# dusk-network/dusk-blindbidproof

Hardware: AMD Instinct MI355X
Metric: blind-bid proofs/sec (higher is better)
Workload: dtype u32

## Files before the change

__graft_entry__.py:

```python
import os
import shutil
import subprocess
import sys

ROOT = os.path.dirname(os.path.abspath(__file__))
PKG = os.path.join(ROOT, "dusk_blindbidproof_amd")
CSRC = os.path.join(PKG, "csrc")
LIB = os.path.join(PKG, "libbbp_hip.so")
ORACLE_SO = os.path.join(ROOT, "oracle", "_build", "libbbp_oracle.so")
HOSTCHECK_SO = os.path.join(ROOT, "tests", "_build", "libhostcheck.so")
DEVCHECK_SO = {"chain": os.path.join(ROOT, "tests", "_build", "libbbp_devcheck.so"),
               "nochain": os.path.join(ROOT, "tests", "_build", "libbbp_devcheck_nochain.so")}
DEVCHECK_DEFS = {"chain": [], "nochain": ["-DBBP_FE_NO_CHAIN"]}


def _newer(target, sources):
    if not os.path.exists(target):
        return True
    t = os.path.getmtime(target)
    return any(os.path.getmtime(s) > t for s in sources)


def _run(cmd):
    print("+", " ".join(cmd), flush=True)
# ... 169 lines not shown
    src = os.path.join(ROOT, "tests", "wire_fuzz.cpp")
    sdir = os.path.join(PKG, "server")
    if force or _newer(WIRE_FUZZ_BIN, [src, os.path.join(sdir, "wire.h"), os.path.join(sdir, "tlv.h")]):
        os.makedirs(os.path.dirname(WIRE_FUZZ_BIN), exist_ok=True)
        _run(["g++", "-O1", "-g", "-std=c++17", "-fsanitize=address,undefined", "-fno-sanitize-recover=all", "-o", WIRE_FUZZ_BIN, src])
    return WIRE_FUZZ_BIN


VERIFY_PLAN_SAN_BIN = os.path.join(ROOT, "tests", "_build", "verify_plan_san")


def build_verify_plan_san(force=False):
    src = os.path.join(ROOT, "tests", "verify_plan_san.cpp")
    if force or _newer(VERIFY_PLAN_SAN_BIN, [src, os.path.join(ROOT, "tests", "host_check.cpp")] + _csrc_files((".h", ".inc"))):
        os.makedirs(os.path.dirname(VERIFY_PLAN_SAN_BIN), exist_ok=True)
        _run(["g++", "-O1", "-g", "-std=c++17", "-fsanitize=address,undefined", "-fno-sanitize-recover=all", "-o", VERIFY_PLAN_SAN_BIN, src])
    return VERIFY_PLAN_SAN_BIN


BATCH_LAYOUT_SAN_BIN = os.path.join(ROOT, "tests", "_build", "batch_layout_san")


def build_batch_layout_san(force=False):
    src = os.path.join(ROOT, "tests", "batch_layout_san.cpp")
    if force or _newer(BATCH_LAYOUT_SAN_BIN, [src, os.path.join(ROOT, "tests", "host_check.cpp")] + _csrc_files((".h", ".inc"))):
        os.makedirs(os.path.dirname(BATCH_LAYOUT_SAN_BIN), exist_ok=True)
        _run(["g++", "-O1", "-g", "-std=c++17", "-fsanitize=address,undefined", "-fno-sanitize-recover=all", "-o", BATCH_LAYOUT_SAN_BIN, src])
    return BATCH_LAYOUT_SAN_BIN


HEDGE_SAN_BIN = os.path.join(ROOT, "tests", "_build", "hedge_san")


def build_hedge_san(force=False):
    src = os.path.join(ROOT, "tests", "hedge_san.cpp")
    if force or _newer(HEDGE_SAN_BIN, [src] + _csrc_files((".h", ".inc"))):
        os.makedirs(os.path.dirname(HEDGE_SAN_BIN), exist_ok=True)
        _run(["g++", "-O1", "-g", "-std=c++17", "-fsanitize=address,undefined", "-fno-sanitize-recover=all", "-o", HEDGE_SAN_BIN, src])
    return HEDGE_SAN_BIN


TAIL_SHARE_BIN = os.path.join(ROOT, "tests", "_build", "tail_share_check")


def build_tail_share_check(force=False):
    src = os.path.join(ROOT, "tests", "tail_share_check.cpp")
    if force or _newer(TAIL_SHARE_BIN, [src] + _csrc_files((".h", ".inc"))):
        os.makedirs(os.path.dirname(TAIL_SHARE_BIN), exist_ok=True)
        _run(["g++", "-O1", "-g", "-std=c++17", "-fsanitize=address,undefined", "-fno-sanitize=signed-integer-overflow,shift", "-fno-sanitize-recover=all", "-o",
              TAIL_SHARE_BIN, src])
    return TAIL_SHARE_BIN


SECRET_MAP_BIN = os.path.join(ROOT, "tests", "_build", "secret_map_check")
SECRET_WIPE_SAN_BIN = os.path.join(ROOT, "tests", "_build", "secret_wipe_san")


def build_secret_map_check(force=False):
    src = os.path.join(ROOT, "tests", "secret_map_check.cpp")
    if force or _newer(SECRET_MAP_BIN, [src] + _csrc_files((".h", ".inc"))):
        os.makedirs(os.path.dirname(SECRET_MAP_BIN), exist_ok=True)
        _run(["g++", "-O1", "-g", "-std=c++17", "-fsanitize=address,undefined", "-fno-sanitize-recover=all", "-o", SECRET_MAP_BIN, src])
    return SECRET_MAP_BIN


ROUND_SELECT_BIN = os.path.join(ROOT, "tests", "_build", "round_select_check")


def build_round_select_check(force=False):
    src = os.path.join(ROOT, "tests", "round_select_check.cpp")
    if force or _newer(ROUND_SELECT_BIN, [src] + _csrc_files((".h", ".inc")) + [os.path.join(ROOT, "include", "bbp.h")]):
        os.makedirs(os.path.dirname(ROUND_SELECT_BIN), exist_ok=True)
        _run(["g++", "-O1", "-g", "-std=c++17", "-fsanitize=address,undefined", "-fno-sanitize-recover=all", "-o", ROUND_SELECT_BIN, src])
    return ROUND_SELECT_BIN


ROUND_BEST_BIN = os.path.join(ROOT, "tests", "_build", "round_best_check")


def build_round_best_check(force=False):
    src = os.path.join(ROOT, "tests", "round_best_check.cpp")
    if force or _newer(ROUND_BEST_BIN, [src] + _csrc_files((".h", ".inc")) + [os.path.join(ROOT, "include", "bbp.h")]):
        os.makedirs(os.path.dirname(ROUND_BEST_BIN), exist_ok=True)
        _run(["g++", "-O1", "-g", "-std=c++17", "-fsanitize=address,undefined", "-fno-sanitize-recover=all", "-o", ROUND_BEST_BIN, src])
    return ROUND_BEST_BIN


ROUNDS_BEST_BIN = os.path.join(ROOT, "tests", "_build", "rounds_best_check")


def build_rounds_best_check(force=False):
    src = os.path.join(ROOT, "tests", "rounds_best_check.cpp")
    if force or _newer(ROUNDS_BEST_BIN, [src] + _csrc_files((".h", ".inc")) + [os.path.join(ROOT, "include", "bbp.h")]):
        os.makedirs(os.path.dirname(ROUNDS_BEST_BIN), exist_ok=True)
        _run(["g++", "-O1", "-g", "-std=c++17", "-fsanitize=address,undefined", "-fno-sanitize-recover=all", "-o", ROUNDS_BEST_BIN, src])
    return ROUNDS_BEST_BIN


ROUND_BEST_DISTINCT_BIN = os.path.join(ROOT, "tests", "_build", "round_best_distinct_check")


def build_round_best_distinct_check(force=False):
    src = os.path.join(ROOT, "tests", "round_best_distinct_check.cpp")
    if force or _newer(ROUND_BEST_DISTINCT_BIN, [src] + _csrc_files((".h", ".inc")) + [os.path.join(ROOT, "include", "bbp.h")]):
        os.makedirs(os.path.dirname(ROUND_BEST_DISTINCT_BIN), exist_ok=True)
        _run(["g++", "-O1", "-g", "-std=c++17", "-fsanitize=address,undefined", "-fno-sanitize-recover=all", "-o", ROUND_BEST_DISTINCT_BIN, src])
# ... 66 lines not shown
COMBINER_RULES_BIN = os.path.join(ROOT, "tests", "_build", "combiner_rules")


def build_combiner_rules(force=False):
    srcs = [os.path.join(ROOT, "tests", "combiner_rules.cpp"), os.path.join(CSRC, "submit.cpp")]
    if force or _newer(COMBINER_RULES_BIN, srcs + [os.path.join(CSRC, "submit.h")]):
        os.makedirs(os.path.dirname(COMBINER_RULES_BIN), exist_ok=True)
        _run(["g++", "-O1", "-std=c++17", "-pthread", "-o", COMBINER_RULES_BIN] + srcs)
    return COMBINER_RULES_BIN


COMBINER_MIXED_BIN = {False: os.path.join(ROOT, "tests", "_build", "combiner_mixed"), True: os.path.join(ROOT, "tests", "_build", "combiner_mixed_tsan")}


def build_combiner_mixed(tsan=False, force=False):
    out = COMBINER_MIXED_BIN[bool(tsan)]
    srcs = [os.path.join(ROOT, "tests", "combiner_mixed.cpp"), os.path.join(CSRC, "submit.cpp")]
    if force or _newer(out, srcs + [os.path.join(CSRC, "submit.h")]):
        os.makedirs(os.path.dirname(out), exist_ok=True)
        flags = ["-O1", "-g", "-fsanitize=thread"] if tsan else ["-O1"]
        _run(["g++"] + flags + ["-std=c++17", "-pthread", "-o", out] + srcs)
    return out


COMBINER_ROUNDS_BIN = {False: os.path.join(ROOT, "tests", "_build", "combiner_rounds"), True: os.path.join(ROOT, "tests", "_build", "combiner_rounds_tsan")}


def build_combiner_rounds(tsan=False, force=False):
    out = COMBINER_ROUNDS_BIN[bool(tsan)]
    srcs = [os.path.join(ROOT, "tests", "combiner_rounds.cpp"), os.path.join(CSRC, "submit.cpp")]
    if force or _newer(out, srcs + [os.path.join(CSRC, "submit.h")]):
        os.makedirs(os.path.dirname(out), exist_ok=True)
        flags = ["-O1", "-g", "-fsanitize=thread"] if tsan else ["-O1"]
        _run(["g++"] + flags + ["-std=c++17", "-pthread", "-o", out] + srcs)
    return out


def build():
    build_hip()
    build_server()
    build_stub_engine()
    build_oracle()
    build_hostcheck()
    build_sortcheck()
    build_roundcheck()
    build_round_select_check()
    build_round_best_check()
    build_round_best_distinct_check()
    build_rounds_best_check()
    build_rounds_best_distinct_check()
    build_round_standing_check()
    build_standings_check()
    build_tail_share_check()
    build_devcheck_all()
    sys.path.insert(0, ROOT)
    import dusk_blindbidproof_amd


def smoke():
    sys.path.insert(0, ROOT)
    import dusk_blindbidproof_amd as bbp
    from tests import smoke_case

    smoke_case.run(bbp)


if __name__ == "__main__":
    build()
```

dusk_blindbidproof_amd/csrc/keccak.h:

```cpp
#pragma once
#include "field.h"

namespace bbp {

BBP_HD u64 rotl64(u64 x, int n) {
    n &= 63;
    if (n == 0) return x;
#if defined(__HIP_DEVICE_COMPILE__)
    const u32 lo = (u32)x, hi = (u32)(x >> 32);
    if (n == 32) return ((u64)lo << 32) | hi;
    const u32 a = n < 32 ? lo : hi, b = n < 32 ? hi : lo;
    const u32 s = 32u - ((u32)n & 31u);
    const u32 rl = __builtin_amdgcn_alignbit(a, b, s), rh = __builtin_amdgcn_alignbit(b, a, s);
    return ((u64)rh << 32) | rl;
#else
    return (x << n) | (x >> (64 - n));
#endif
}

#define BBP_BITOP3_XOR3 0x96
#define BBP_BITOP3_CHI 0xd2
BBP_HD u64 keccak_xor3(u64 a, u64 b, u64 c) {
#if defined(__HIP_DEVICE_COMPILE__)
    const u32 lo = __builtin_amdgcn_bitop3_b32((u32)a, (u32)b, (u32)c, BBP_BITOP3_XOR3);
// ... 179 lines not shown
BBP_HD void merlin_challenge(merlin_transcript& t, const uint8_t* label, u32 llen, uint8_t* out, u32 n) {
    uint8_t len4[4];
    le32(len4, n);
    strobe_meta_ad(t, label, llen, false);
    strobe_meta_ad(t, len4, 4, true);
    strobe_prf(t, out, n, false);
}

BBP_HD void merlin_rng_rekey(merlin_transcript& t, const uint8_t* label, u32 llen, const uint8_t* w, u32 wlen) {
    uint8_t len4[4];
    le32(len4, wlen);
    strobe_meta_ad(t, label, llen, false);
    strobe_meta_ad(t, len4, 4, true);
    strobe_key(t, w, wlen, false);
}

BBP_HD void merlin_rng_finalize(merlin_transcript& t, const uint8_t* ent32) {
    const uint8_t l[3] = {'r', 'n', 'g'};
    strobe_meta_ad(t, l, 3, false);
    strobe_key(t, ent32, 32, false);
}

BBP_HD void merlin_rng_fill(merlin_transcript& t, uint8_t* out, u32 n) {
    uint8_t len4[4];
    le32(len4, n);
    strobe_meta_ad(t, len4, 4, false);
    strobe_prf(t, out, n, false);
}

BBP_HD bool merlin_rng_fill64_bulk(merlin_transcript& t, u32 count, u32* out_words ) {
    if (t.pos != 64 || t.pos_begin != 0) return false;
    u64 a[25];
#pragma unroll
    for (int i = 0; i < 25; i++) a[i] = t.st[i];
    for (u32 c = 0; c < count; c++) {
        a[8] ^= 0x0741000000401200ull;
        a[9] ^= 0x0000000000000447ull;
        a[20] ^= 0x8000000000000000ull;
        keccak_f1600_body(a);
        u32* o = out_words + (size_t)c * 16;
#pragma unroll
        for (int i = 0; i < 8; i++) {
            o[2 * i] = (u32)a[i];
            o[2 * i + 1] = (u32)(a[i] >> 32);
            a[i] = 0;
        }
    }
#pragma unroll
    for (int i = 0; i < 25; i++) t.st[i] = a[i];
    t.cur_flags = BBP_FLAG_I | BBP_FLAG_A | BBP_FLAG_C;
    return true;
}

}
```

dusk_blindbidproof_amd/csrc/prove_plan.h:

```cpp
#pragma once
#include <stdint.h>
#include <stdio.h>
#include <stdlib.h>
#include <string.h>

#include <string>

namespace bbp {

constexpr int FOLD_ROUND = 7;
constexpr int PROVE_MAX_SLICES = 4;
#ifndef BBP_PROVE_BUFS
#define BBP_PROVE_BUFS 5
#endif
constexpr int PROVE_BUFS = BBP_PROVE_BUFS;

struct ProveKnobs {
    int slices = 3;
    int rotate_below = 1023;
    int rotate_deep_max = 4096;
    int deep_from = 3;
    int mixed_from = 512;
    int dual_open_below = 1024;
    int rng_coop = -1;
    int rng_coop_below = 768;
    int rng_coop_idle_below = 2300;
    int rng_dpp = 2;
    int rng_block = 0;
    int serial_block = 64;
    int serial_lds = 160 * 1024;
    int tr_wave_below = 32;
    int ipa_wide_below = 32;
    int commit_split_below = 1024;
    int witness_native = 1;
    int tail_small_below = 65;
    int tail_round = FOLD_ROUND;
    int stagger_mode = 0;
    int trace_prove = 0;
    int open_on_chain = -1;
    int hw_queues = 4;

    struct Env {
        const char* name;
        int ProveKnobs::*member;
        int (*clamp)(int);
    };
    template <class F>
    static void each_env(F&& f) {
        static const Env table[] = {
            {"BBP_SLICES", &ProveKnobs::slices, [](int v) { return v < 1 ? 1 : v > PROVE_MAX_SLICES ? PROVE_MAX_SLICES : v; }},
            {"BBP_ROTATE_BELOW", &ProveKnobs::rotate_below, nullptr},
            {"BBP_ROTATE_DEEP_MAX", &ProveKnobs::rotate_deep_max, nullptr},
            {"BBP_ROTATE_DEEP_FROM", &ProveKnobs::deep_from, [](int v) { return v < 2 ? 2 : v; }},
            {"BBP_ROTATE_MIXED_FROM", &ProveKnobs::mixed_from, nullptr},
            {"BBP_DUAL_OPEN_BELOW", &ProveKnobs::dual_open_below, nullptr},
            {"BBP_RNG_COOP", &ProveKnobs::rng_coop, [](int v) { return v != 0 ? 1 : 0; }},
            {"BBP_RNG_COOP_BELOW", &ProveKnobs::rng_coop_below, nullptr},
            {"BBP_RNG_COOP_IDLE_BELOW", &ProveKnobs::rng_coop_idle_below, nullptr},
            {"BBP_RNG_DPP", &ProveKnobs::rng_dpp, nullptr},
            {"BBP_RNG_BLOCK", &ProveKnobs::rng_block, [](int v) { return v >= 1024 ? 1024 : v >= 512 ? 512 : v >= 256 ? 256 : v >= 128 ? 128 : 64; }},
            {"BBP_SERIAL_BLOCK", &ProveKnobs::serial_block, [](int v) { return v == 64 ? 64 : v == 128 ? 128 : 256; }},
            {"BBP_SERIAL_LDS", &ProveKnobs::serial_lds, [](int v) { return v < 0 ? 0 : v > 160 * 1024 ? 160 * 1024 : v; }},
            {"BBP_TR_WAVE_BELOW", &ProveKnobs::tr_wave_below, nullptr},
            {"BBP_IPA_WIDE_BELOW", &ProveKnobs::ipa_wide_below, nullptr},
            {"BBP_COMMIT_SPLIT_BELOW", &ProveKnobs::commit_split_below, nullptr},
            {"BBP_WITNESS_NATIVE", &ProveKnobs::witness_native, [](int v) { return v != 0 ? 1 : 0; }},
            {"BBP_TAIL_SMALL_BELOW", &ProveKnobs::tail_small_below, nullptr},
            {"BBP_TAIL_ROUND", &ProveKnobs::tail_round, [](int v) { return v == FOLD_ROUND ? FOLD_ROUND : 12; }},
// ... 35 lines not shown

struct HeavyPlan {
    uint32_t tw = 0;
    uint32_t tgrid = 0;
    bool wide_ipa = false;
    bool split_T = false;
    uint32_t tail_from = 12;
    int stagger_after = 0;
};

inline HeavyPlan plan_heavy(const ProveKnobs& k, uint32_t B) {
    HeavyPlan h;
    h.tw = B <= (uint32_t)k.tr_wave_below ? 1u : 0u;
    h.tgrid = h.tw ? B : (B + 63) / 64;
    h.wide_ipa = B <= (uint32_t)k.ipa_wide_below;
    h.split_T = B * 5 <= (uint32_t)k.commit_split_below;
    h.tail_from = B < (uint32_t)(k.tail_small_below > 0 ? k.tail_small_below : 0) ? 12u : (uint32_t)k.tail_round;
    h.stagger_after = k.stagger_mode;
    return h;
}

enum StreamRole { ROLE_CALLER = 0, ROLE_SIDE, ROLE_LANE1, ROLE_LANE2, ROLE_LANE3, ROLE_COPY, ROLE_SIDE2, ROLE_COUNT };

struct ProvePlan {
    enum Chain { SERIAL, LANES25, WORD, HALFWORD };
    uint32_t call = 0;
    bool deep = false;
    bool behind_sliced = false;
    bool dual = false;
    int open_stream = 0;
    int par = 0;
    bool coop = false;
    Chain chain = SERIAL;
    uint32_t prefix_form = 0;
    uint32_t serial_blk = 64;
    uint32_t cblk = 64;
    bool rotate = false;
    int heavy_stream = 0;
    uint32_t slices = 0;
    bool open_on_chain = false;
    int chain_stream = -1;

    int open_role() const { return open_on_chain ? chain_stream : open_stream ? ROLE_SIDE2 : ROLE_SIDE; }
    int heavy_role() const { return open_on_chain ? chain_stream : ROLE_LANE1 + heavy_stream - 1; }
    static int slice_role(uint32_t i) { return i == 0 ? ROLE_CALLER : ROLE_LANE1 + (int)i - 1; }
    uint32_t roles() const {
        uint32_t mask = 1u << ROLE_CALLER | 1u << open_role();
        if (rotate) mask |= 1u << heavy_role();
        for (uint32_t i = 0; i < slices; i++) mask |= 1u << slice_role(i);
        return mask;
    }
    int raw_index() const { return !open_on_chain ? open_stream : chain_stream == ROLE_SIDE ? 0 : 1 + heavy_stream; }
    uint32_t cblk_wave() const { return 2 * cblk > 1024u ? 1024u : 2 * cblk; }
    uint32_t slice_first(uint32_t B, uint32_t i) const { return (uint32_t)(((uint64_t)B * i) / slices); }

    std::string trace_line(uint32_t call_, uint32_t B, int inflight) const {
        char buf[160];
        snprintf(buf, sizeof buf, "prove call %u: B %u inflight %d deep %d behind_sliced %d dual %d rotate %d par %d coop %d\n", call_, B, inflight,
                 (int)deep, (int)behind_sliced, (int)dual, (int)rotate, par, (int)coop);
        return buf;
    }
};

template <class Busy>
ProvePlan plan_prove(const ProveKnobs& k, ProveRuleState& st, uint32_t B, int inflight, Busy&& sliced_busy) {
    ProvePlan p;
    p.call = st.calls++;
    if (inflight >= k.deep_from) {
        st.deep_mode = true;
        st.deep_idle_seen = 0;
    } else if (++st.deep_idle_seen >= 6) {
        st.deep_mode = false;
    }
    p.deep = (st.deep_mode || st.force_deep) && k.deep_eligible(B);
    p.behind_sliced = !p.deep && k.mixed_from > 0 && B >= (uint32_t)k.mixed_from && st.last_sliced && sliced_busy();
    p.dual = !p.behind_sliced && (p.deep || B < (uint32_t)(k.dual_open_below > 0 ? k.dual_open_below : 0));
    p.open_stream = p.dual ? (int)(p.call & 1u) : 0;
    p.par = p.dual ? (int)(p.call % (uint32_t)PROVE_BUFS) : (int)(p.call & 1u);
    p.coop = k.rng_coop < 0 ? B <= (uint32_t)k.rng_coop_below || (inflight == 0 && B <= (uint32_t)k.rng_coop_idle_below) : k.rng_coop != 0;
    p.chain = !p.coop ? ProvePlan::SERIAL : k.rng_dpp >= 2 ? ProvePlan::HALFWORD : k.rng_dpp ? ProvePlan::WORD : ProvePlan::LANES25;
    p.prefix_form = !p.coop ? 0u : B <= (uint32_t)k.tr_wave_below ? 2u : 1u;
    p.serial_blk = k.serial_lds > 0 ? (uint32_t)k.serial_block : 64u;
    p.cblk = k.rng_block > 0 ? (uint32_t)k.rng_block : (B <= 128 ? 64u : B <= 256 ? 128u : 256u);
    p.rotate = p.dual && ((k.rotate_below > 0 && B <= (uint32_t)k.rotate_below) || (p.deep && B > (uint32_t)k.rotate_below));
    p.heavy_stream = p.rotate ? 1 + (int)(p.call % (uint32_t)(PROVE_MAX_SLICES - 1)) : 0;
    p.slices = B >= 64u * (uint32_t)k.slices ? (uint32_t)k.slices : (B >= 128 ? 2u : 1u);
    if (p.dual && p.slices > 2) p.slices = 2;
    if (p.rotate) p.slices = 0;
    p.open_on_chain = p.rotate && k.chain_rule(p.deep);
    p.chain_stream = !p.open_on_chain ? -1 : p.heavy_stream == 3 ? (int)ROLE_SIDE : (int)ROLE_LANE1 + p.heavy_stream - 1;
    return p;
}

}
```

dusk_blindbidproof_amd/csrc/prover.hip:

```cpp
#define BBP_KECCAK_WAVE 1
#include <string.h>

#include <functional>

#include "batch.h"
#include "hosthash.h"
#include "keccak_wave.h"
#include "scalarmul.h"
#include "witness.h"

namespace bbp {

#define BBP_THIN_PRIO() __builtin_amdgcn_s_setprio(3)
#ifndef BBP_LANE_KERNEL
#define BBP_LANE_KERNEL __launch_bounds__(64)
#endif


__device__ __forceinline__ void sc_to_bytes32(uint8_t* o, const sc& s) { sc_tobytes(o, s); }
__device__ __forceinline__ void words_to_bytes32(uint8_t* o, const u32* w) {
#pragma unroll
    for (int i = 0; i < 8; i++) {
        o[4 * i] = (uint8_t)w[i];
        o[4 * i + 1] = (uint8_t)(w[i] >> 8);
// ... 118 lines not shown
    out[(size_t)p * out_stride + c] = acc;
}

__global__ BBP_LANE_KERNEL void k_commit_split(u32 count, u32 per_proof, const sc* __restrict__ values, const sc* __restrict__ blindings, u32 stride_v,
                                               u32 stride_b, const niels_packed* __restrict__ comb, ge* __restrict__ out, u32 out_stride) {
    const u32 t = blockIdx.x * blockDim.x + threadIdx.x, g = t / COMMIT_L, q = t % COMMIT_L;
    const u32 gi = g < count ? g : count - 1;
    const u32 p = gi / per_proof, c = gi % per_proof;
    const sc v = ld_sc(&values[(size_t)p * stride_v + c]);
    const sc b = ld_sc(&blindings[(size_t)p * stride_b + c]);
    ge acc = comb_mul_add_part(ge_identity(), comb, v, q);
    acc = comb_mul_add_part(acc, comb + 64 * 8, b, q);
    acc = commit_group_sum(acc);
    if (q == 0 && g < count) out[(size_t)p * out_stride + c] = acc;
}

int32_t commit_launch(bbp_ctx* ctx, u32 count, const sc* values, const sc* blindings, u32 stride_v, u32 stride_b, u32 per_proof,
                      ge* out, u32 out_stride, hipStream_t s) {
    if (!count) return BBP_OK;
    ScopedEvent ev(ctx, TAG_COMMIT, s);
    if (count <= (u32)ctx->knobs.commit_split_below) {
        hipLaunchKernelGGL(k_commit_split, dim3((count * COMMIT_L + 63) / 64), dim3(64), 0, s, count, per_proof, values, blindings, stride_v, stride_b,
                           ctx->comb, out, out_stride);
        BBP_HIP_TRY(ctx, hipGetLastError());
        return BBP_OK;
    }
    hipLaunchKernelGGL(k_commit, dim3((count + 63) / 64), dim3(64), 0, s, count, per_proof, values, blindings, stride_v, stride_b,
                       ctx->comb, out, out_stride);
    BBP_HIP_TRY(ctx, hipGetLastError());
    return BBP_OK;
}

#ifdef BBP_ENCODE_WAVES
#define BBP_ENCODE_ATTR __attribute__((amdgpu_waves_per_eu(BBP_ENCODE_WAVES, BBP_ENCODE_WAVES)))
#else
#define BBP_ENCODE_ATTR
#endif
__global__ BBP_LANE_KERNEL BBP_ENCODE_ATTR void k_encode_strided(u32 count, u32 per_proof, const ge* __restrict__ pts, u32 pts_stride, u32* __restrict__ enc,
                                 u32 enc_stride_words, u32 enc_off_words, u32 pts_cstride) {
    BBP_THIN_PRIO();
    u32 t = blockIdx.x * blockDim.x + threadIdx.x;
    if (t >= count) return;
    u32 p = t / per_proof, c = t % per_proof;
    u32 w[8];
    ge_encode_words(w, pts[(size_t)p * pts_stride + (size_t)c * pts_cstride]);
    u32* o = enc + (size_t)p * enc_stride_words + enc_off_words + 8 * c;
#pragma unroll
    for (int i = 0; i < 8; i++) o[i] = w[i];
}


__device__ void tr_open_lane(u32 p, u32 m, u32 n1, const merlin_transcript& prefix, const u32* __restrict__ enc, const u8* __restrict__ entropy,
                             const sc* __restrict__ vb_all, u32* __restrict__ raw, merlin_transcript* __restrict__ tr_out,
                             merlin_transcript* __restrict__ rng_out, bool coop, u32 wave) {
    merlin_transcript t = prefix;
    t.wave = wave;
    const u32* e = enc + (size_t)p * enc_words(m);
    for (u32 i = 0; i < m; i++) tr_append_words(t, LBL("V"), e + enc_V(i));
    merlin_append_u64(t, LBL("m"), (u64)m);
    merlin_transcript r = t;
    const sc* vb = vb_all + (size_t)p * m;
    for (u32 i = 0; i < m; i++) {
        uint8_t b[32];
        sc_to_bytes32(b, ld_sc(&vb[i]));
        merlin_rng_rekey(r, LBL("v_blinding"), b, 32);
    }
    const u8* ent = entropy + (size_t)p * (32 * (size_t)m + 32) + 32 * (size_t)m;
    uint8_t seed[32];
    for (int i = 0; i < 32; i++) seed[i] = ent[i];
    merlin_rng_finalize(r, seed);
    u32* rw = raw + (size_t)p * (3 + 2 * (size_t)n1) * 16;
    {
        uint8_t b[64];
        merlin_rng_fill(r, b, 64);
        bytes_to_words(rw, b, 16);
    }
    if (!coop) merlin_rng_fill64_bulk(r, 2 + 2 * n1, rw + 16);
    t.wave = r.wave = 0;
    tr_out[p] = t;
    rng_out[p] = r;
}

__global__ void k_open_serial(u32 B, u32 rng_blocks, u32 m, u32 n1, merlin_transcript prefix, const u32* __restrict__ enc,
                              const u8* __restrict__ entropy, const sc* __restrict__ vb_all, u32* __restrict__ raw,
                              merlin_transcript* __restrict__ tr_out, merlin_transcript* __restrict__ rng_out, u32 n_cst,
                              const u32* __restrict__ w_terms, const u32* __restrict__ w_loff, const u32* __restrict__ w_roff,
                              const sc* __restrict__ cst_all, const sc* __restrict__ v_all, sc* __restrict__ ai1_all, sc* __restrict__ ao1_all,
                              u32 coop) {
    if (blockIdx.x < rng_blocks) {
        const u32 t = blockIdx.x * blockDim.x + threadIdx.x, p = coop == 2 ? t >> 6 : t;
        if (p < B) tr_open_lane(p, m, n1, prefix, enc, entropy, vb_all, raw, tr_out, rng_out, coop != 0, coop == 2);
    } else {
        const u32 p = (blockIdx.x - rng_blocks) * blockDim.x + threadIdx.x;
        if (p < B) witness_gates_lane(p, m, n1, n_cst, w_terms, w_loff, w_roff, cst_all, v_all, ai1_all, ao1_all);
    }
}

__device__ __forceinline__ u64 coop_gather64(int addr, u64 v) {
    const u32 lo = (u32)__builtin_amdgcn_ds_bpermute(addr, (int)(u32)v);
    const u32 hi = (u32)__builtin_amdgcn_ds_bpermute(addr, (int)(u32)(v >> 32));
    return ((u64)hi << 32) | lo;
}

struct coop_lane {
    int col[4], dm, dp, s0, s1, s2;
    u32 rot;
    u64 iota_mask;
};

__device__ __forceinline__ coop_lane coop_setup(u32 lane_in_wave) {
    const u32 l = lane_in_wave & 31u, base = lane_in_wave & 32u;
    const u32 li = l < 25 ? l : 0;
    const u32 x = li % 5, y = li / 5;
    const u32 RHO[25] = {0, 1, 62, 28, 27, 36, 44, 6, 55, 20, 3, 10, 43, 25, 39, 41, 45, 15, 21, 8, 18, 2, 61, 56, 14};
    coop_lane c;
#pragma unroll
    for (int k = 0; k < 4; k++) c.col[k] = 4 * (int)(base + x + 5 * ((y + 1 + k) % 5));
    c.dm = 4 * (int)(base + (x + 4) % 5 + 5 * y);
    c.dp = 4 * (int)(base + (x + 1) % 5 + 5 * y);
    auto src = [&](u32 X) { return 4 * (int)(base + (X + 3 * y) % 5 + 5 * X); };
    c.s0 = src(x);
    c.s1 = src((x + 1) % 5);
    c.s2 = src((x + 2) % 5);
    c.rot = RHO[li];
    c.iota_mask = l == 0 ? ~0ull : 0ull;
    return c;
}

__device__ __forceinline__ u64 coop_keccak_f(u64 a, const coop_lane& c) {
    const u64 RC[24] = {0x0000000000000001ull, 0x0000000000008082ull, 0x800000000000808Aull, 0x8000000080008000ull,
                        0x000000000000808Bull, 0x0000000080000001ull, 0x8000000080008081ull, 0x8000000000008009ull,
                        0x000000000000008Aull, 0x0000000000000088ull, 0x0000000080008009ull, 0x000000008000000Aull,
                        0x000000008000808Bull, 0x800000000000008Bull, 0x8000000000008089ull, 0x8000000000008003ull,
                        0x8000000000008002ull, 0x8000000000000080ull, 0x000000000000800Aull, 0x800000008000000Aull,
                        0x8000000080008081ull, 0x8000000000008080ull, 0x0000000080000001ull, 0x8000000080008008ull};
#pragma unroll 1
    for (int r = 0; r < 24; r++) {
        const u64 C = a ^ coop_gather64(c.col[0], a) ^ coop_gather64(c.col[1], a) ^ coop_gather64(c.col[2], a) ^ coop_gather64(c.col[3], a);
        const u64 Cm = coop_gather64(c.dm, C), Cp = coop_gather64(c.dp, C);
        a ^= Cm ^ ((Cp << 1) | (Cp >> 63));
        const u64 ro = (a << c.rot) | (a >> ((64u - c.rot) & 63u));
        const u64 b0 = coop_gather64(c.s0, ro), b1 = coop_gather64(c.s1, ro), b2 = coop_gather64(c.s2, ro);
        a = b0 ^ (~b1 & b2);
        a ^= RC[r] & c.iota_mask;
// ... 924 lines not shown
    if ((rc = guard.enter())) return rc;
    int inflight = 0;
    for (int k = 0; k < bbp_ctx::CALL_RING; k++)
        if (ctx->ev_call_valid[k] && hipEventQuery(ctx->ev_call[k]) == hipErrorNotReady) inflight++;
    const ProvePlan plan = plan_prove(ctx->knobs, ctx->prove_state, B, inflight, [&] {
        const int lp = ctx->last_prove_par;
        return lp >= 0 && ctx->ev_done_valid[lp] && hipEventQuery(ctx->ev_done[lp]) == hipErrorNotReady;
    });
    const int ridx = plan.raw_index(), par = plan.par;
    if (plan.open_role() == ROLE_SIDE2 && !ctx->side2) BBP_HIP_TRY(ctx, hipStreamCreateWithFlags(&ctx->side2, hipStreamNonBlocking));
    BatchDev bd;
    const BatchDims dims = c.dims();
    if ((rc = batch_reserve(ctx, B, dims, bd, par))) return rc;
    const BatchStrides st = batch_strides(dims);
    const u32 m = c.m, n1 = c.n_mul;
    const merlin_transcript prefix = prover_prefix();
    const size_t n_draws = 3 + 2 * (size_t)n1;
    if ((rc = dev_reserve(ctx, ctx->raw[ridx], (size_t)B * n_draws * 64))) return rc;
    u32* const raw = (u32*)ctx->raw[ridx].p;
    BBP_HIP_TRY(ctx, hipEventRecord(ctx->ev_entry[par], s));
    hipStream_t os = role_stream(ctx, plan.open_role(), s);
    if (plan.chain_stream == ROLE_SIDE) BBP_HIP_TRY(ctx, hipStreamWaitEvent(os, ctx->ev_join[3], 0));
    if (ctx->ev_done_valid[par]) BBP_HIP_TRY(ctx, hipStreamWaitEvent(os, ctx->ev_done[par], 0));
    if (ctx->ev_prep_valid) {
        BBP_HIP_TRY(ctx, hipStreamWaitEvent(os, ctx->ev_prep, 0));
        ctx->ev_prep_valid = false;
    }
    if (ctx->ev_draw_valid) {
        BBP_HIP_TRY(ctx, hipStreamWaitEvent(os, ctx->ev_draw, 0));
        ctx->ev_draw_valid = false;
    }
    if (open_hook && (rc = (*open_hook)(os))) return rc;
    LAUNCH(ctx, TAG_WITNESS, k_fill_mimc, cdiv(B * BBP_MIMC_ROUNDS, 64), 64, os, B, c.n_cst, ctx->mimc_c, bd.cst);
    u32 hog = 0;
    if ((rc = serial_lds_bytes(ctx, (const void*)k_open_serial, &hog))) return rc;
    LAUNCH(ctx, TAG_WITNESS, k_witness_head, cdiv(B, 64), 64, os, B, N, c.n_cst, in_dev, bd.cst, bd.v);
    LAUNCH(ctx, TAG_TRANSCRIPT, k_load_blindings, cdiv(B * m, 64), 64, os, B, m, ent_dev, bd.vb);
    if ((rc = commit_launch(ctx, B * m, bd.v, bd.vb, st.v, st.vb, m, bd.pts, st.pts, os))) return rc;
    LAUNCH(ctx, TAG_ENCODE, k_encode_strided, cdiv(B * m, 64), 64, os, B * m, m, bd.pts, st.pts, bd.enc, st.enc, enc_V(0), 1u);
    if (plan.coop) {
        const u32 pgrid = plan.prefix_form == 2 ? B : cdiv(B, 64);
        LAUNCH(ctx, TAG_RNG, k_open_serial, pgrid, 64, os, B, pgrid, m, n1, prefix, bd.enc, ent_dev, bd.vb, raw, bd.tr, bd.rng, c.n_cst, c.w_terms,
               c.w_loff, c.w_roff, bd.cst, bd.v, bd.ai1, bd.ao1, plan.prefix_form);
    }
    auto bulk = [&](decltype(&k_open_bulk) kern, u32 lanes, u32 blk) -> int32_t {
        u32 hogb = 0;
        if (int32_t rc = serial_lds_bytes(ctx, (const void*)kern, &hogb)) return rc;
        const u32 nb_rng = cdiv(B * lanes, blk), nb_wit = cdiv(B, blk);
        LAUNCH_LDS(ctx, TAG_RNG, kern, nb_rng + nb_wit, blk, hogb, os, B, nb_rng, n1, 2 + 2 * n1, bd.rng, raw, m, c.n_cst, c.w_terms, c.w_loff,
                   c.w_roff, bd.cst, bd.v, bd.ai1, bd.ao1, hogb, (u32)ctx->knobs.witness_native);
        return BBP_OK;
    };
    switch (plan.chain) {
        case ProvePlan::SERIAL:
            LAUNCH_LDS(ctx, TAG_RNG, k_open_serial, 2 * cdiv(B, plan.serial_blk), plan.serial_blk, hog, os, B, cdiv(B, plan.serial_blk), m, n1, prefix,
                       bd.enc, ent_dev, bd.vb, raw, bd.tr, bd.rng, c.n_cst, c.w_terms, c.w_loff, c.w_roff, bd.cst, bd.v, bd.ai1, bd.ao1, 0u);
            break;
        case ProvePlan::LANES25: rc = bulk(k_open_bulk, 32, plan.cblk); break;
        case ProvePlan::WORD: rc = bulk(k_open_bulk8, 64, plan.cblk_wave()); break;
        case ProvePlan::HALFWORD: rc = bulk(k_open_bulk50, 64, plan.cblk_wave()); break;
    }
    if (rc) return rc;
    LAUNCH(ctx, TAG_RNG, k_reduce_draws, cdiv((u32)(B * n_draws), 128), 128, os, B, n1, (const u32*)raw, bd.ai1, bd.ao1, bd.s1,
           plan.chain == ProvePlan::HALFWORD ? 1u : 0u);
    if (wipe_on(ctx)) {
        WipeList wl;
        wipe_take(wl, ctx->raw[ridx]);
        if ((rc = wipe_enqueue(ctx, wl, os))) return rc;
    }
    BBP_HIP_TRY(ctx, hipEventRecord(ctx->ev_open[par], os));
    ctx->ev_open_valid[par] = true;
    if (ctx->knobs.trace_prove) fputs(plan.trace_line(plan.call, B, inflight).c_str(), stderr);
    const size_t rec = BBP_R1CS_PROOF_BYTES + 32 * (size_t)m;
    if (plan.rotate) {
        const int hs = plan.heavy_stream;
        hipStream_t ls = role_stream(ctx, plan.heavy_role(), s);
        if (!plan.open_on_chain) BBP_HIP_TRY(ctx, hipStreamWaitEvent(ls, ctx->ev_open[par], 0));
        if (!plan.open_on_chain && hs == 3) BBP_HIP_TRY(ctx, hipStreamWaitEvent(ls, ctx->ev_join[3], 0));
        if ((rc = prove_heavy(ctx, plan_heavy(ctx->knobs, B), c, bd, B, out_dev, ls, hs, nullptr, ctx->ev_entry[par]))) return rc;
        BBP_HIP_TRY(ctx, hipEventRecord(ctx->ev_join[hs], ls));
        BBP_HIP_TRY(ctx, hipStreamWaitEvent(s, ctx->ev_join[hs], 0));
    }
    for (u32 i = 0; i < plan.slices; i++) {
        const u32 first = plan.slice_first(B, i), last = plan.slice_first(B, i + 1);
        hipStream_t ls = role_stream(ctx, ProvePlan::slice_role(i), s);
        if (i == 3) BBP_HIP_TRY(ctx, hipStreamWaitEvent(ls, ctx->ev_join[3], 0));
        BBP_HIP_TRY(ctx, hipStreamWaitEvent(ls, ctx->ev_open[par], 0));
        const HeavyPlan hp = plan_heavy(ctx->knobs, last - first);
        if (i && hp.stagger_after) BBP_HIP_TRY(ctx, hipStreamWaitEvent(ls, ctx->ev_stagger[i - 1], 0));
        if ((rc = prove_heavy(ctx, hp, c, batch_view(bd, dims, first), last - first, out_dev + rec * first, ls, (int)i,
                              i + 1 < plan.slices ? ctx->ev_stagger[i] : nullptr, i ? ctx->ev_entry[par] : nullptr)))
            return rc;
        if (i) {
            BBP_HIP_TRY(ctx, hipEventRecord(ctx->ev_join[i], ls));
            BBP_HIP_TRY(ctx, hipStreamWaitEvent(s, ctx->ev_join[i], 0));
        }
    }
    if (wipe_on(ctx)) {
        WipeList wl;
        wipe_take(wl, ctx->batch[par]);
        if ((rc = wipe_enqueue(ctx, wl, s))) return rc;
    }
    BBP_HIP_TRY(ctx, hipEventRecord(ctx->ev_done[par], s));
    ctx->ev_done_valid[par] = true;
    ctx->last_par = par;
    ctx->prove_state.last_sliced = !plan.rotate;
    ctx->last_prove_par = par;
    BBP_HIP_TRY(ctx, hipEventRecord(ctx->ev_call[plan.call % (u32)bbp_ctx::CALL_RING], s));
    ctx->ev_call_valid[plan.call % (u32)bbp_ctx::CALL_RING] = true;
    return BBP_OK;
// ... 16 lines not shown
```

Baseline: 24740.

## Split serial Keccak RNG chain across lane pairs using 32-bit halves

The serial open path now runs each proof's bulk RNG Keccak fill on two adjacent lanes. Each lane holds the low or high 32-bit half of the state and swaps halves with its partner through DPP for theta and rho. This is meant to halve the per-lane latency of the long serial Keccak chain, which matters at small batch sizes. In exchange it doubles the threads in the RNG blocks, adds about 30 DPP exchanges per round, and duplicates the transcript prefix work on both lanes. The witness block count is recomputed for the larger block size.

```diff
diff --git a/__graft_entry__.py b/__graft_entry__.py
--- a/__graft_entry__.py
+++ b/__graft_entry__.py
@@ -245,6 +245,27 @@
     return TAIL_SHARE_BIN
 
 
+KECCAK_PAIR_BIN = os.path.join(ROOT, "tests", "_build", "keccak_pair_check")
+DEVCHECK_PAIR_SO = os.path.join(ROOT, "tests", "_build", "libbbp_devcheck_pair.so")
+
+
+def build_keccak_pair_check(force=False):
+    src = os.path.join(ROOT, "tests", "keccak_pair_check.cpp")
+    if force or _newer(KECCAK_PAIR_BIN, [src] + _csrc_files((".h", ".inc"))):
+        os.makedirs(os.path.dirname(KECCAK_PAIR_BIN), exist_ok=True)
+        _run(["g++", "-O1", "-g", "-std=c++17", "-fsanitize=address,undefined", "-fno-sanitize-recover=all", "-o", KECCAK_PAIR_BIN, src])
+    return KECCAK_PAIR_BIN
+
+
+def build_devcheck_pair(force=False):
+    src = os.path.join(ROOT, "tests", "device_check_pair.hip")
+    if force or _newer(DEVCHECK_PAIR_SO, [src] + _csrc_files((".h", ".inc"))):
+        os.makedirs(os.path.dirname(DEVCHECK_PAIR_SO), exist_ok=True)
+        hipcc = shutil.which("hipcc") or "/opt/rocm/bin/hipcc"
+        _run([hipcc, "--offload-arch=gfx950", "-O3", "-std=c++17", "-fPIC", "-shared", src, "-o", DEVCHECK_PAIR_SO])
+    return DEVCHECK_PAIR_SO
+
+
 SECRET_MAP_BIN = os.path.join(ROOT, "tests", "_build", "secret_map_check")
 SECRET_WIPE_SAN_BIN = os.path.join(ROOT, "tests", "_build", "secret_wipe_san")
 
@@ -417,7 +438,9 @@
     build_round_standing_check()
     build_standings_check()
     build_tail_share_check()
+    build_keccak_pair_check()
     build_devcheck_all()
+    build_devcheck_pair()
     sys.path.insert(0, ROOT)
     import dusk_blindbidproof_amd
 
diff --git a/dusk_blindbidproof_amd/csrc/keccak.h b/dusk_blindbidproof_amd/csrc/keccak.h
--- a/dusk_blindbidproof_amd/csrc/keccak.h
+++ b/dusk_blindbidproof_amd/csrc/keccak.h
@@ -255,4 +255,165 @@
     return true;
 }
 
-}
+BBP_HD u32 keccak_alignbit(u32 a, u32 b, u32 s) {
+#if defined(__HIP_DEVICE_COMPILE__)
+    return __builtin_amdgcn_alignbit(a, b, s);
+#else
+    return (u32)(((((u64)a) << 32) | b) >> s);
+#endif
+}
+BBP_HD u32 keccak_xor3_32(u32 a, u32 b, u32 c) {
+#if defined(__HIP_DEVICE_COMPILE__)
+    return __builtin_amdgcn_bitop3_b32(a, b, c, BBP_BITOP3_XOR3);
+#else
+    return (u32)keccak_xor3(a, b, c);
+#endif
+}
+BBP_HD u32 keccak_chi_32(u32 a, u32 b, u32 c) {
+#if defined(__HIP_DEVICE_COMPILE__)
+    return __builtin_amdgcn_bitop3_b32(a, b, c, BBP_BITOP3_CHI);
+#else
+    return (u32)keccak_chi(a, b, c);
+#endif
+}
+#define BBP_PAIR_IOTA_TABLE 0x78
+BBP_HD u32 keccak_xorand_32(u32 a, u32 b, u32 c) {
+#if defined(__HIP_DEVICE_COMPILE__)
+    return __builtin_amdgcn_bitop3_b32(a, b, c, BBP_PAIR_IOTA_TABLE);
+#else
+    return a ^ (b & c);
+#endif
+}
+BBP_HD u32 keccak_pair_rotl(u32 own, u32 partner, int r) { return r < 32 ? keccak_alignbit(own, partner, 32u - (u32)r) : keccak_alignbit(partner, own, 64u - (u32)r); }
+
+BBP_HD void keccak_pair_parity(const u32* a, u32* c) {
+#pragma unroll
+    for (int x = 0; x < 5; x++) c[x] = keccak_xor3_32(keccak_xor3_32(a[x], a[x + 5], a[x + 10]), a[x + 15], a[x + 20]);
+}
+BBP_HD void keccak_pair_theta(u32* a, const u32* c, const u32* pc) {
+#pragma unroll
+    for (int x = 0; x < 5; x++) {
+        const u32 cm = c[(x + 4) % 5], rp = keccak_pair_rotl(c[(x + 1) % 5], pc[(x + 1) % 5], 1);
+#pragma unroll
+        for (int y = 0; y < 5; y++) a[x + 5 * y] = keccak_xor3_32(a[x + 5 * y], cm, rp);
+    }
+}
+BBP_HD void keccak_pair_rho_pi_chi(u32* a, const u32* pa) {
+    u32 b[25];
+    b[0] = a[0];
+#define BBP_KP_RHO(dst, src, r) b[dst] = keccak_pair_rotl(a[src], pa[src], r)
+    BBP_KP_RHO(10, 1, 1); BBP_KP_RHO(20, 2, 62); BBP_KP_RHO(5, 3, 28); BBP_KP_RHO(15, 4, 27);
+    BBP_KP_RHO(16, 5, 36); BBP_KP_RHO(1, 6, 44); BBP_KP_RHO(11, 7, 6); BBP_KP_RHO(21, 8, 55); BBP_KP_RHO(6, 9, 20);
+    BBP_KP_RHO(7, 10, 3); BBP_KP_RHO(17, 11, 10); BBP_KP_RHO(2, 12, 43); BBP_KP_RHO(12, 13, 25); BBP_KP_RHO(22, 14, 39);
+    BBP_KP_RHO(23, 15, 41); BBP_KP_RHO(8, 16, 45); BBP_KP_RHO(18, 17, 15); BBP_KP_RHO(3, 18, 21); BBP_KP_RHO(13, 19, 8);
+    BBP_KP_RHO(14, 20, 18); BBP_KP_RHO(24, 21, 2); BBP_KP_RHO(9, 22, 61); BBP_KP_RHO(19, 23, 56); BBP_KP_RHO(4, 24, 14);
+#undef BBP_KP_RHO
+#pragma unroll
+    for (int y = 0; y < 25; y += 5) {
+#pragma unroll
+        for (int x = 0; x < 5; x++) a[y + x] = keccak_chi_32(b[y + x], b[y + (x + 1) % 5], b[y + (x + 2) % 5]);
+    }
+}
+BBP_HD void keccak_pair_iota(u32* a, u32 sel, int r) {
+#define BBP_KP_RC(hi, lo) (((u64)((hi) ^ (lo)) << 32) | (lo))
+    const u64 RC[24] = {BBP_KP_RC(0x00000000u, 0x00000001u), BBP_KP_RC(0x00000000u, 0x00008082u), BBP_KP_RC(0x80000000u, 0x0000808Au),
+                        BBP_KP_RC(0x80000000u, 0x80008000u), BBP_KP_RC(0x00000000u, 0x0000808Bu), BBP_KP_RC(0x00000000u, 0x80000001u),
+                        BBP_KP_RC(0x80000000u, 0x80008081u), BBP_KP_RC(0x80000000u, 0x00008009u), BBP_KP_RC(0x00000000u, 0x0000008Au),
+                        BBP_KP_RC(0x00000000u, 0x00000088u), BBP_KP_RC(0x00000000u, 0x80008009u), BBP_KP_RC(0x00000000u, 0x8000000Au),
+                        BBP_KP_RC(0x00000000u, 0x8000808Bu), BBP_KP_RC(0x80000000u, 0x0000008Bu), BBP_KP_RC(0x80000000u, 0x00008089u),
+                        BBP_KP_RC(0x80000000u, 0x00008003u), BBP_KP_RC(0x80000000u, 0x00008002u), BBP_KP_RC(0x80000000u, 0x00000080u),
+                        BBP_KP_RC(0x00000000u, 0x0000800Au), BBP_KP_RC(0x80000000u, 0x8000000Au), BBP_KP_RC(0x80000000u, 0x80008081u),
+                        BBP_KP_RC(0x80000000u, 0x00008080u), BBP_KP_RC(0x00000000u, 0x80000001u), BBP_KP_RC(0x80000000u, 0x80008008u)};
+#undef BBP_KP_RC
+    const u64 k = RC[r];
+    a[0] = keccak_xorand_32(a[0], sel, (u32)(k >> 32)) ^ (u32)k;
+}
+
+#if defined(__HIPCC__)
+__device__ __forceinline__ u32 keccak_pair_partner(u32 v) { return (u32)__builtin_amdgcn_update_dpp(0, (int)v, 0xb1, 0xf, 0xf, true); }
+
+__device__ __forceinline__ void keccak_f1600_pair(u32* a, u32 sel) {
+    for (int r = 0; r < 24; r++) {
+        u32 c[5], pc[5], pa[25];
+        keccak_pair_parity(a, c);
+#pragma unroll
+        for (int x = 0; x < 5; x++) pc[x] = keccak_pair_partner(c[x]);
+        keccak_pair_theta(a, c, pc);
+        pa[0] = 0;
+#pragma unroll
+        for (int i = 1; i < 25; i++) pa[i] = keccak_pair_partner(a[i]);
+        keccak_pair_rho_pi_chi(a, pa);
+        keccak_pair_iota(a, sel, r);
+    }
+}
+#endif
+
+inline void keccak_f1600_pair_model(u32* lo, u32* hi) {
+    for (int r = 0; r < 24; r++) {
+        u32 cl[5], ch[5], pl[25], ph[25];
+        keccak_pair_parity(lo, cl);
+        keccak_pair_parity(hi, ch);
+        keccak_pair_theta(lo, cl, ch);
+        keccak_pair_theta(hi, ch, cl);
+        for (int i = 0; i < 25; i++) pl[i] = lo[i], ph[i] = hi[i];
+        keccak_pair_rho_pi_chi(lo, ph);
+        keccak_pair_rho_pi_chi(hi, pl);
+        keccak_pair_iota(lo, 0u, r);
+        keccak_pair_iota(hi, ~0u, r);
+    }
+}
+
+BBP_HD void merlin_pair_draw_framing(u32* a, u32 sel) {
+    a[8] ^= sel ? 0x07410000u : 0x00401200u;
+    a[9] ^= sel ? 0u : 0x00000447u;
+    a[20] ^= sel ? 0x80000000u : 0u;
+}
+
+#if defined(__HIPCC__)
+__device__ __forceinline__ bool merlin_rng_fill64_bulk_pair(merlin_transcript& t, u32 count, u32* out_words , u32 odd) {
+    if (t.pos != 64 || t.pos_begin != 0) return false;
+    const u32 sel = odd ? ~0u : 0u;
+    u32 a[25];
+#pragma unroll
+    for (int i = 0; i < 25; i++) a[i] = odd ? (u32)(t.st[i] >> 32) : (u32)t.st[i];
+    for (u32 c = 0; c < count; c++) {
+        merlin_pair_draw_framing(a, sel);
+        keccak_f1600_pair(a, sel);
+        u32* o = out_words + (size_t)c * 16 + odd;
+#pragma unroll
+        for (int i = 0; i < 8; i++) {
+            o[2 * i] = a[i];
+            a[i] = 0;
+        }
+    }
+#pragma unroll
+    for (int i = 0; i < 25; i++) {
+        const u32 q = keccak_pair_partner(a[i]);
+        t.st[i] = odd ? ((u64)a[i] << 32) | q : ((u64)q << 32) | a[i];
+    }
+    t.cur_flags = BBP_FLAG_I | BBP_FLAG_A | BBP_FLAG_C;
+    return true;
+}
+#endif
+
+inline bool merlin_rng_fill64_bulk_pair_model(merlin_transcript& t, u32 count, u32* out_words ) {
+    if (t.pos != 64 || t.pos_begin != 0) return false;
+    u32 lo[25], hi[25];
+    for (int i = 0; i < 25; i++) lo[i] = (u32)t.st[i], hi[i] = (u32)(t.st[i] >> 32);
+    for (u32 c = 0; c < count; c++) {
+        merlin_pair_draw_framing(lo, 0u);
+        merlin_pair_draw_framing(hi, ~0u);
+        keccak_f1600_pair_model(lo, hi);
+        u32* o = out_words + (size_t)c * 16;
+        for (int i = 0; i < 8; i++) {
+            o[2 * i] = lo[i];
+            o[2 * i + 1] = hi[i];
+            lo[i] = hi[i] = 0;
+        }
+    }
+    for (int i = 0; i < 25; i++) t.st[i] = ((u64)hi[i] << 32) | lo[i];
+    t.cur_flags = BBP_FLAG_I | BBP_FLAG_A | BBP_FLAG_C;
+    return true;
+}
+
+}
diff --git a/dusk_blindbidproof_amd/csrc/prove_plan.h b/dusk_blindbidproof_amd/csrc/prove_plan.h
--- a/dusk_blindbidproof_amd/csrc/prove_plan.h
+++ b/dusk_blindbidproof_amd/csrc/prove_plan.h
@@ -14,6 +14,10 @@
 #define BBP_PROVE_BUFS 5
 #endif
 constexpr int PROVE_BUFS = BBP_PROVE_BUFS;
+#ifndef BBP_SERIAL_PAIR
+#define BBP_SERIAL_PAIR 1
+#endif
+constexpr uint32_t SERIAL_CHAIN_LANES = BBP_SERIAL_PAIR ? 2 : 1;
 
 struct ProveKnobs {
     int slices = 3;
@@ -155,6 +159,7 @@
     }
     int raw_index() const { return !open_on_chain ? open_stream : chain_stream == ROLE_SIDE ? 0 : 1 + heavy_stream; }
     uint32_t cblk_wave() const { return 2 * cblk > 1024u ? 1024u : 2 * cblk; }
+    uint32_t serial_chain_lanes() const { return SERIAL_CHAIN_LANES * serial_blk; }
     uint32_t slice_first(uint32_t B, uint32_t i) const { return (uint32_t)(((uint64_t)B * i) / slices); }
 
     std::string trace_line(uint32_t call_, uint32_t B, int inflight) const {
diff --git a/dusk_blindbidproof_amd/csrc/prover.hip b/dusk_blindbidproof_amd/csrc/prover.hip
--- a/dusk_blindbidproof_amd/csrc/prover.hip
+++ b/dusk_blindbidproof_amd/csrc/prover.hip
@@ -194,7 +194,8 @@
 
 __device__ void tr_open_lane(u32 p, u32 m, u32 n1, const merlin_transcript& prefix, const u32* __restrict__ enc, const u8* __restrict__ entropy,
                              const sc* __restrict__ vb_all, u32* __restrict__ raw, merlin_transcript* __restrict__ tr_out,
-                             merlin_transcript* __restrict__ rng_out, bool coop, u32 wave) {
+                             merlin_transcript* __restrict__ rng_out, bool coop, u32 wave, u32 pair_lane) {
+    const bool writer = pair_lane != 2;
     merlin_transcript t = prefix;
     t.wave = wave;
     const u32* e = enc + (size_t)p * enc_words(m);
@@ -215,10 +216,15 @@
     {
         uint8_t b[64];
         merlin_rng_fill(r, b, 64);
-        bytes_to_words(rw, b, 16);
-    }
+        if (writer) bytes_to_words(rw, b, 16);
+    }
+#if BBP_SERIAL_PAIR
+    if (!coop) merlin_rng_fill64_bulk_pair(r, 2 + 2 * n1, rw + 16, pair_lane == 2 ? 1u : 0u);
+#else
     if (!coop) merlin_rng_fill64_bulk(r, 2 + 2 * n1, rw + 16);
+#endif
     t.wave = r.wave = 0;
+    if (!writer) return;
     tr_out[p] = t;
     rng_out[p] = r;
 }
@@ -230,8 +236,9 @@
                               const sc* __restrict__ cst_all, const sc* __restrict__ v_all, sc* __restrict__ ai1_all, sc* __restrict__ ao1_all,
                               u32 coop) {
     if (blockIdx.x < rng_blocks) {
-        const u32 t = blockIdx.x * blockDim.x + threadIdx.x, p = coop == 2 ? t >> 6 : t;
-        if (p < B) tr_open_lane(p, m, n1, prefix, enc, entropy, vb_all, raw, tr_out, rng_out, coop != 0, coop == 2);
+        const u32 t = blockIdx.x * blockDim.x + threadIdx.x, pair = BBP_SERIAL_PAIR && coop == 0 ? 1u + (t & 1u) : 0u;
+        const u32 p = coop == 2 ? t >> 6 : pair ? t >> 1 : t;
+        if (p < B) tr_open_lane(p, m, n1, prefix, enc, entropy, vb_all, raw, tr_out, rng_out, coop != 0, coop == 2, pair);
     } else {
         const u32 p = (blockIdx.x - rng_blocks) * blockDim.x + threadIdx.x;
         if (p < B) witness_gates_lane(p, m, n1, n_cst, w_terms, w_loff, w_roff, cst_all, v_all, ai1_all, ao1_all);
@@ -1262,10 +1269,12 @@
         return BBP_OK;
     };
     switch (plan.chain) {
-        case ProvePlan::SERIAL:
-            LAUNCH_LDS(ctx, TAG_RNG, k_open_serial, 2 * cdiv(B, plan.serial_blk), plan.serial_blk, hog, os, B, cdiv(B, plan.serial_blk), m, n1, prefix,
-                       bd.enc, ent_dev, bd.vb, raw, bd.tr, bd.rng, c.n_cst, c.w_terms, c.w_loff, c.w_roff, bd.cst, bd.v, bd.ai1, bd.ao1, 0u);
+        case ProvePlan::SERIAL: {
+            const u32 blk = plan.serial_chain_lanes(), nb_rng = cdiv(B, plan.serial_blk), nb_wit = cdiv(B, blk);
+            LAUNCH_LDS(ctx, TAG_RNG, k_open_serial, nb_rng + nb_wit, blk, hog, os, B, nb_rng, m, n1, prefix, bd.enc, ent_dev, bd.vb, raw, bd.tr, bd.rng,
+                       c.n_cst, c.w_terms, c.w_loff, c.w_roff, bd.cst, bd.v, bd.ai1, bd.ao1, 0u);
             break;
+        }
         case ProvePlan::LANES25: rc = bulk(k_open_bulk, 32, plan.cblk); break;
         case ProvePlan::WORD: rc = bulk(k_open_bulk8, 64, plan.cblk_wave()); break;
         case ProvePlan::HALFWORD: rc = bulk(k_open_bulk50, 64, plan.cblk_wave()); break;
```

New measurement: 25460, median of 6. +2.9%, better.
